# tungphambasement/DCNN

Measured on AMD Instinct MI355X. Metric: images/sec (whole node) ResNet-18 Tiny-ImageNet training at 1/2/4/8 MI355X, higher is better.
Workload: dtype bf16; 1 GPU; model=resnet18_tiny_imagenet, global_batch=256, per_gpu_batch=256, parallelism=dp1, optimizer=adam, hipgraph=True, engine=native (C++ host API)

## Files before the change

dcnn_amd/csrc/host/ops_gpu.hip:

```cpp
#include <hip/hip_runtime.h>

#include <algorithm>
#include <cmath>
#include <cstdio>
#include <cstdlib>
#include <cstring>
#include <map>
#include <mutex>
#include <stdexcept>
#include <string>
#include <unordered_map>
#include <vector>

#include "../kernels/api.h"
#include "dcnn/ops.hpp"
#include "dcnn/tensor.hpp"

#define HOST_HIP_CHECK(x)                                                                    \
  do {                                                                                       \
    hipError_t e_ = (x);                                                                     \
    if (e_ != hipSuccess) throw std::runtime_error(std::string(#x) + ": " + hipGetErrorString(e_)); \
  } while (0)

namespace dcnn {
// ... 739 lines not shown
  const GcArgs g = gc_args(s, groups);
  const int splits = dcnn::gconv_wgrad_splits(kBF16, g);
  wgrad_split(splits, (long)s.Co * s.KH * s.KW * (s.C / groups), s.Co, gw, gb,
              [&](float* slab, float* bslab) { dcnn::gconv_wgrad(kBF16, dy, x, slab, bslab, g, cur()); });
}

bool stem_ok(const ConvShape& s) {
  return s.KH == 3 && s.KW == 3 && s.SH == 1 && s.SW == 1 && s.PH == 1 && s.PW == 1 &&
         stem_supported(s.N, s.C, s.H, s.W, s.Co);
}

const float* stem_fwd(const float* x, const void* w, const float* bias, void* y, const ConvShape& s, int* stat_rows) {
  rec("stem_fwd", s, -1, {{"bias", bias != nullptr}, {"stats", stat_rows != nullptr}});
  StemArgs a{};
  a.x = x; a.w = w; a.w_bf16 = 1;
  a.ws[0] = 9l * s.C; a.ws[1] = 1; a.ws[2] = 3l * s.C; a.ws[3] = s.C;
  a.bias = bias; a.y = static_cast<bf16*>(y);
  a.N = s.N; a.Ci = s.C; a.H = s.H; a.W = s.W; a.Co = s.Co;
  if (stat_rows) {
    *stat_rows = stem_tiles_host(s.N, s.H, s.W);
    a.slab = static_cast<float*>(scratch(fwd_stats_slot(), (size_t)*stat_rows * 3 * s.Co * 4));
  }
  dcnn::stem_fwd(a, cur());
  return a.slab;
}

static void stem_wgrad_impl(const void* dy, const float* x, float* gw, float* gb, const ConvShape& s,
                            const StemBn* bn);

void stem_wgrad(const void* dy, const float* x, float* gw, float* gb, const ConvShape& s) {
  stem_wgrad_impl(dy, x, gw, gb, s, nullptr);
}

static std::pair<const float*, int> reduce_stats(int mode, const float* slab, int rows, int C);

void stem_wgrad_bn(const void* dy, const float* x, float* gw, float* gb, const ConvShape& s, const StemBn& bn) {
  stem_wgrad_impl(dy, x, gw, gb, s, &bn);
}

static void stem_wgrad_impl(const void* dy, const float* x, float* gw, float* gb, const ConvShape& s,
                            const StemBn* bn) {
  rec("stem_wgrad", s, -1, {{"bias", gb != nullptr}, {"deferred", g_defer}, {"bn", bn != nullptr}});
  std::pair<const float*, int> st{nullptr, 0};
  if (bn) st = reduce_stats(1, bn->slab, bn->rows, s.Co);
  const int blocks = bn ? stem_wgrad_blocks_bnt(s.N, s.H, s.W) : stem_wgrad_blocks(s.N, s.H, s.W);
  const long n = 9l * s.C * s.Co;
  wgrad_split(blocks, n, s.Co, gw, gb, [&](float* slab, float* bslab) {
    StemArgs a{};
    a.x = x; a.dy = static_cast<const bf16*>(dy); a.slab = slab; a.bias_slab = bslab;
    a.gs[0] = 9l * s.C; a.gs[1] = 1; a.gs[2] = 3l * s.C; a.gs[3] = s.C;
    a.n_slab = n;
    a.N = s.N; a.Ci = s.C; a.H = s.H; a.W = s.W; a.Co = s.Co;
    if (bn) {
      a.bn_x = static_cast<const bf16*>(bn->x); a.bn_mean = bn->mean; a.bn_istd = bn->istd; a.bn_gamma = bn->gamma;
      a.bn_sums = st.first; a.bn_parts = st.second; a.bn_count = (float)((long)s.N * s.H * s.W);
      a.bn_dgamma = bn->dgamma; a.bn_dbeta = bn->dbeta; a.bn_eval = bn->train ? 0 : 1;
    }
    dcnn::stem_wgrad(a, blocks, cur());
  });
}

void dense_fwd(const void* x, const void* w, const float* bias, void* y, int N, int In, int Out) {
  NtArgs a{static_cast<const bf16*>(x), static_cast<const bf16*>(w), y, N, Out, In, In, In, Out, kPlain, 0, 0, 0, 0,
           1, 1, 1, 1, 1, 1, 0, 0, bias, nullptr, nullptr, 0, 0};
  gemm_nt(a, cur());
}

void dense_dgrad(const void* dy, const void* w, void* dx, int N, int In, int Out) {
  bf16* wt = static_cast<bf16*>(scratch(W_T, (size_t)In * Out * 2));
  conv_weight_transpose(kBF16, w, wt, Out, 1, In, cur());
  NtArgs a{static_cast<const bf16*>(dy), wt, dx, N, In, Out, Out, Out, In, kPlain, 0, 0, 0, 0, 1, 1, 1, 1, 1, 1, 0, 0,
           nullptr, nullptr, nullptr, 0, 0};
  gemm_nt(a, cur());
}

void dense_wgrad(const void* dy, const void* x, float* gw, float* gb, int N, int In, int Out) {
  const int splits = gemm_tn_splits(Out, In, N);
  wgrad_split(splits, (long)Out * In, Out, gw, gb, [&](float* slab, float* bslab) {
    TnArgs a{static_cast<const bf16*>(dy), static_cast<const bf16*>(x), slab, bslab, Out, In, N, kPlain, 0, 0, 0, 0,
             1, 1, 1, 1, 1, 1, 0, 0, In, 0};
    gemm_tn(a, splits, cur());
  });
}

bool head_supported(const PoolShape& p, int Out) { return dcnn::head_supported(geom(p), Out); }

void head_fwd(const void* x, const void* w, const float* bias, void* pooled, void* y, const PoolShape& p, int Out) {
  dcnn::head_fwd(static_cast<const bf16*>(x), static_cast<const bf16*>(w), bias, static_cast<bf16*>(pooled),
                 static_cast<bf16*>(y), geom(p), Out, cur());
}

void head_bwd(const void* dy, const void* w, const void* pooled, void* dx, float* gw, float* gb, const PoolShape& p,
              int Out) {
  wgrad_split(head_bwd_splits(p.N, p.C, Out), (long)Out * p.C, Out, gw, gb, [&](float* slab, float* bslab) {
    dcnn::head_bwd(static_cast<const bf16*>(dy), static_cast<const bf16*>(w), static_cast<const bf16*>(pooled),
                   static_cast<bf16*>(dx), slab, bslab, geom(p), Out, cur());
  });
}

static std::pair<const float*, int> reduce_stats(int mode, const float* slab, int rows, int C) {
  const int parts = bn_stat_parts(rows);
  float* sums = static_cast<float*>(scratch(STAT_SUMS, (size_t)2 * C * 4));
  float* part = parts > 1 ? static_cast<float*>(scratch(STAT_PART, (size_t)parts * 3 * C * 4)) : nullptr;
  bn_stat_reduce(mode, slab, rows, C, sums, part, nullptr, cur());
  return {parts > 1 ? part : sums, parts};
}

void bn_fwd(const void* x, void* y, long R, int C, const float* g, const float* b, float eps, bool train,
            float* rmean, float* rvar, float momentum, float* smean, float* sistd, bool relu, const void* residual) {
  if (!train) {
    bn_apply(kBF16, x, y, R, C, nullptr, 1, (float)R, g, b, eps, residual, relu ? 1 : 0, smean, sistd, rmean, rvar,
             momentum, 1, cur());
    return;
  }
  const int rows = bn_partial_rows(R, C);
  float* slab = static_cast<float*>(scratch(STAT_SLAB, (size_t)rows * 3 * C * 4));
  bn_partial(kBF16, x, nullptr, nullptr, nullptr, nullptr, nullptr, R, C, slab, 0, nullptr, cur());
  const auto st = reduce_stats(0, slab, rows, C);
  bn_apply(kBF16, x, y, R, C, st.first, st.second, (float)R, g, b, eps, residual, relu ? 1 : 0, smean, sistd, rmean,
           rvar, momentum, 0, cur());
}

void bn_fwd_slab(const void* x, void* y, long R, int C, const float* slab, int rows, const float* g, const float* b,
                 float eps, float* rmean, float* rvar, float momentum, float* smean, float* sistd, bool relu,
                 const void* residual) {
  const auto st = reduce_stats(0, slab, rows, C);
  bn_apply(kBF16, x, y, R, C, st.first, st.second, (float)R, g, b, eps, residual, relu ? 1 : 0, smean, sistd, rmean,
           rvar, momentum, 0, cur());
}

void bn_bwd_slab(const void* dy, const void* x, void* dx, long R, int C, const float* mean, const float* istd,
                 const float* g, float* dg, float* db, bool train, const float* slab, int rows) {
  const auto st = reduce_stats(1, slab, rows, C);
  bn_bwd_apply(kBF16, dy, nullptr, x, dx, R, C, mean, istd, g, st.first, st.second, (float)R, dg, db, train ? 0 : 1, cur());
}

void bn_bwd(const void* dy, const void* x, void* dx, long R, int C, const float* mean, const float* istd,
            const float* g, float* dg, float* db, bool train, const void* yout, void* dy_out) {
  const int rows = bn_partial_rows(R, C);
  float* slab = static_cast<float*>(scratch(STAT_SLAB, (size_t)rows * 2 * C * 4));
  bn_partial(kBF16, x, dy, yout, dy_out, mean, istd, R, C, slab, 1, nullptr, cur());
  const auto st = reduce_stats(1, slab, rows, C);
  bn_bwd_apply(kBF16, dy, yout, x, dx, R, C, mean, istd, g, st.first, st.second, (float)R, dg, db, train ? 0 : 1, cur());
}

SecondaryStats::SecondaryStats() { t_secondary = true; }
SecondaryStats::~SecondaryStats() { t_secondary = false; }

BnRaw bn_stats_raw(const void* x, long R, int C, const float* slab, int rows) {
  if (slab != nullptr && rows > 0) return BnRaw{slab, rows};
  const int n = bn_partial_rows(R, C);
  float* s = static_cast<float*>(scratch(STAT_SLAB2, (size_t)n * 3 * C * 4));
  bn_partial(kBF16, x, nullptr, nullptr, nullptr, nullptr, nullptr, R, C, s, 0, nullptr, cur());
  return BnRaw{s, n};
}

bool bn_dual_ok(long R, int C) { return bn_apply_dual_supported(R, C); }

static void reduce_pair(int mode, const float* slab_a, int rows_a, const float* slab_b, int rows_b, int C,
                        std::pair<const float*, int>& a, std::pair<const float*, int>& b) {
  const int pa = bn_stat_parts(rows_a), pb = bn_stat_parts(rows_b);
  float* sa = static_cast<float*>(scratch(STAT_SUMS, (size_t)2 * C * 4));
  float* sb = static_cast<float*>(scratch(STAT_SUMS2, (size_t)2 * C * 4));
  float* qa = pa > 1 ? static_cast<float*>(scratch(STAT_PART, (size_t)pa * 3 * C * 4)) : nullptr;
  float* qb = pb > 1 ? static_cast<float*>(scratch(STAT_PART2, (size_t)pb * 3 * C * 4)) : nullptr;
  bn_stat_reduce2(mode, slab_a, rows_a, sa, qa, slab_b, rows_b, sb, qb, C, cur());
  a = {pa > 1 ? qa : sa, pa};
  b = {pb > 1 ? qb : sb, pb};
}

void bn_fwd_dual(const BnFwdSide& a, const BnFwdSide& b, void* y, long R, int C, bool relu, bool train) {
  std::pair<const float*, int> sa{nullptr, 1}, sb{nullptr, 1};
  if (train) reduce_pair(0, a.raw.slab, a.raw.rows, b.raw.slab, b.raw.rows, C, sa, sb);
  auto side = [&](const BnFwdSide& s, const std::pair<const float*, int>& st) {
    return BnSide{s.x,     st.first, st.second, (float)R, s.g,        s.b,    s.eps,
                  s.smean, s.sistd,  s.rmean,   s.rvar,   s.momentum, train ? 0 : 1};
  };
  if (!bn_apply_dual(side(a, sa), side(b, sb), y, R, C, relu ? 1 : 0, cur()))
    throw std::runtime_error("bn_fwd_dual: unsupported shape");
}

void bn_bwd_dual(const void* dy, const BnBwdSides& a, const float* slab_a, int rows_a, const BnBwdSides& b, long R,
                 int C) {
  const int rows_b = bn_partial_rows(R, C);
  float* slab_b = static_cast<float*>(scratch(STAT_SLAB, (size_t)rows_b * 2 * C * 4));
  bn_partial(kBF16, b.x, dy, nullptr, nullptr, b.mean, b.istd, R, C, slab_b, 1, nullptr, cur());
  std::pair<const float*, int> sa, sb;
  reduce_pair(1, slab_a, rows_a, slab_b, rows_b, C, sa, sb);
  auto side = [&](const BnBwdSides& s, const std::pair<const float*, int>& st) {
    return BnBwdSide{s.x, s.dx, s.mean, s.istd, s.g, st.first, st.second, (float)R, s.dg, s.db};
  };
  if (!bn_bwd_apply_dual(dy, side(a, sa), side(b, sb), R, C, cur()))
    throw std::runtime_error("bn_bwd_dual: unsupported shape");
}

bool bn_relu_maxpool_ok(const PoolShape& p) {
  const PoolGeom g = geom(p);
  return dcnn::bn_relu_maxpool_supported(g) && dcnn::maxpool_bwd_bnb_supported(g);
}

void bn_relu_maxpool(const void* x, void* y, uint8_t* idx, const PoolShape& p, const float* slab, int rows,
                     const float* g, const float* b, float eps, float* rmean, float* rvar, float momentum,
                     float* smean, float* sistd) {
  const long R = (long)p.N * p.H * p.W;
  if (slab == nullptr || rows <= 0) {
    rows = bn_partial_rows(R, p.C);
    float* s = static_cast<float*>(scratch(STAT_SLAB, (size_t)rows * 3 * p.C * 4));
    bn_partial(kBF16, x, nullptr, nullptr, nullptr, nullptr, nullptr, R, p.C, s, 0, nullptr, cur());
    slab = s;
  }
  const auto st = reduce_stats(0, slab, rows, p.C);
  dcnn::bn_relu_maxpool(static_cast<const bf16*>(x), static_cast<bf16*>(y), idx, geom(p), st.first, st.second,
                        (float)R, g, b, eps, smean, sistd, rmean, rvar, momentum, cur());
}

const float* maxpool_bwd_bnb(const void* dy, const uint8_t* idx, const void* ypool, const void* x, const float* mean,
                             const float* istd, void* dx, const PoolShape& p, int* rows) {
  const PoolGeom g = geom(p);
  *rows = maxpool_bwd_bnb_rows(g);
  float* slab = static_cast<float*>(scratch(BWD_STATS, (size_t)*rows * 2 * p.C * 4));
  dcnn::maxpool_bwd_bnb(static_cast<const bf16*>(dy), idx, static_cast<const bf16*>(ypool),
// ... 254 lines not shown
```

dcnn_amd/csrc/kernels/api.h:

```cpp
#pragma once
#include <hip/hip_runtime.h>
#include <stdint.h>

#include "fusion_plan.h"
#include "optim_segments.h"
typedef __bf16 bf16;

namespace dcnn {
struct BnbArgs {
  const bf16* y; const bf16* x; const float* mean; const float* istd;
  const float* gamma; const float* beta; int mask_x;
};
struct NtArgs {
  const bf16* A; const bf16* B; void* C;
  int M, N, K; int lda, ldb, ldc; int mode;
  int nb, sh, sw, cs, gh, gw; int kh, kw, strh, strw, padh, padw;
  const float* bias; const bf16* residual; float* stats; int out_f32; int relu;
};
struct TnArgs {
  const bf16* dY; const bf16* X; float* slab; float* bias_slab;
  int M, N, P; int mode; int nb, sh, sw, cs, gh, gw; int kh, kw, strh, strw, padh, padw; int ldx; int k_per_split;
};
struct G2Args {
  const bf16* A; const bf16* B; bf16* C;
// ... 117 lines not shown
void gemm_t2f(T2Args a, int splits, hipStream_t s);
int gemm_t2f_splits(int M, int N, int P);
void set_f32_mode(int mode);
int get_f32_mode();
void conv_weight_transpose_f32(const float* w, float* wt, int Co, int T_, int Ci, hipStream_t s);
void gemm_tn(TnArgs a, int splits, hipStream_t s);
int gemm_tn_splits(int M, int N, int P);
int gemm_tn_k_per_split(int P, int splits);
int gemm_tn_bias_rows(int M);
struct ConvRouteGeom {
  int N, C, H, W, Co, KH, KW, SH, SW, PH, PW, OH, OW, g1s_mode;
};
enum ConvRoute : int { ROUTE_GENERIC = 0, ROUTE_GEMM_G2 = 1, ROUTE_HALO = 2, ROUTE_G1S = 3, ROUTE_HALO_S2 = 4 };
int conv_fwd_route(ConvRouteGeom g);
int conv_dgrad_route(ConvRouteGeom g);
int conv_wgrad_route(ConvRouteGeom g);
void splitk_reduce(const float* slab, float* out, long n, int splits, int accumulate, hipStream_t s);
void splitk_reduce2(const float* slab, float* out, long n, const float* bslab, float* bout, long nb, int splits,
                    int accumulate, hipStream_t s);

constexpr int kMaxRed = 48;
struct RedEnt { const float* slab; float* out; long n; int splits, unit0, chunks, groups, vec, wpc; };
struct MultiRed { int count; RedEnt e[kMaxRed]; };
void multi_splitk_reduce(MultiRed t, hipStream_t s);

int bn_partial_rows(long R, int C);
void bn_partial(int dtype, const void* x, const void* dy, const void* yout, void* dy_out, const float* mean,
                const float* istd, long R, int C, float* slab, int mode, float* zero_sums, hipStream_t s);
int bn_stat_parts(int rows);
void bn_stat_reduce2(int mode, const float* slab, int rows, float* out, float* part, const float* slab2, int rows2,
                     float* out2, float* part2, int C, hipStream_t s);
void bn_stat_reduce(int mode, const float* slab, int rows, int C, float* out, float* part, unsigned* ticket,
                    hipStream_t s);
void bn_apply(int dtype, const void* x, void* y, long R, int C, const float* sums, int parts, float count, const float* gamma,
              const float* beta, float eps, const void* residual, int relu, float* save_mean, float* save_istd,
              float* run_mean, float* run_var, float momentum, int use_running, hipStream_t s);
struct BnSide {
  const void* x; const float* sums; int parts; float count; const float* gamma; const float* beta; float eps;
  float* save_mean; float* save_istd; float* run_mean; float* run_var; float momentum; int use_running;
};
bool bn_apply_dual(const BnSide& a, const BnSide& b, void* y, long R, int C, int relu, hipStream_t s);
bool bn_apply_dual_supported(long R, int C);
struct BnBwdSide {
  const void* x; void* dx; const float* mean; const float* istd; const float* gamma; const float* sums; int parts;
  float count; float* dgamma; float* dbeta;
};
bool bn_bwd_apply_dual(const void* dy, const BnBwdSide& a, const BnBwdSide& b, long R, int C, hipStream_t s);
void bn_bwd_apply(int dtype, const void* dy, const void* yout, const void* x, void* dx, long R, int C, const float* mean,
                  const float* istd, const float* gamma, const float* sums, int parts, float count, float* dgamma,
                  float* dbeta, int eval_mode, hipStream_t s);
bool bn_relu_maxpool_supported(PoolGeom g);
void bn_relu_maxpool(const bf16* x, bf16* y, uint8_t* idx, PoolGeom g, const float* sums, int parts, float count,
                     const float* gamma, const float* beta, float eps, float* save_mean, float* save_istd,
                     float* run_mean, float* run_var, float momentum, hipStream_t s);
void gn_fwd(int dtype, const void* x, void* y, int N, int HW, int C, int G, const float* gamma, const float* beta,
            float eps, float* save_mean, float* save_istd, hipStream_t s);
void gn_bwd(int dtype, const void* dy, const void* x, void* dx, int N, int HW, int C, int G, const float* gamma,
            const float* mean, const float* istd, float* dgamma, float* dbeta, float* aff, hipStream_t s);
bool ln_supported(int dt, long R, int C);
int ln_partial_rows(long R, int C);
long ln_workspace_bytes(long R, int C);
void ln_fwd(int dt, const void* x, void* y, long R, int C, const float* gamma, const float* beta, float eps,
            float* save_mean, float* save_rstd, hipStream_t s);
void ln_bwd(int dt, const void* dy, const void* x, void* dx, long R, int C, const float* gamma, const float* mean,
            const float* rstd, float* dgamma, float* dbeta, float* workspace, hipStream_t s);
void lscale_fwd(int dt, const void* x, const float* gamma, const void* residual, void* y, long R, int C,
// ... 130 lines not shown
```

dcnn_amd/csrc/kernels/bindings.cpp:

```cpp
#include <tuple>
#include <pybind11/pybind11.h>
#include <pybind11/stl.h>
#include <algorithm>
#include <array>
#include <vector>
#include <hip/hip_runtime.h>
#include <stdint.h>

namespace py = pybind11;
#include "api.h"


using namespace dcnn;
void bind_runtime(py::module_& m);
void bind_rccl(py::module_& m);
template <typename T>
static inline T P(uintptr_t x) { return reinterpret_cast<T>(x); }
static inline hipStream_t S(uintptr_t x) { return reinterpret_cast<hipStream_t>(x); }

using Ptr4 = std::array<uintptr_t, 4>;
static BnbArgs bnb_of(const Ptr4& b) {
  return BnbArgs{P<const bf16*>(b[0]), P<const bf16*>(b[1]), P<const float*>(b[2]), P<const float*>(b[3])};
}

// ... 242 lines not shown
                            unsigned b_bytes, int M, int N, int Pn, int splits, uintptr_t stream) {
    bind_gemm_t2(f32, dY, X, slab, bias_slab, a_bytes, b_bytes, M, N, Pn, M, N, 1, 1, 1, 1, 1, 1, {{0, 0}}, splits, stream);
  });
  m.def("gemm_t2_splits", &gemm_t2_splits);
  m.def("gemm_tn",
        [](uintptr_t dY, uintptr_t X, uintptr_t slab, uintptr_t bias_slab, int M, int N, int Pn, int mode, int nb,
           int sh, int sw, int cs, int gh, int gw, int kh, int kw, int strh, int strw, int padh, int padw, int ldx,
           int splits, uintptr_t stream) {
          TnArgs a{P<const bf16*>(dY), P<const bf16*>(X), P<float*>(slab), P<float*>(bias_slab), M, N, Pn, mode, nb, sh,
                   sw, cs, gh, gw, kh, kw, strh, strw, padh, padw, ldx, 0};
          gemm_tn(a, splits, S(stream));
        });
  m.def("gemm_tn_splits", &gemm_tn_splits);
  m.def("splitk_reduce", [](uintptr_t slab, uintptr_t out, long n, int splits, int acc, uintptr_t st) {
    splitk_reduce(P<const float*>(slab), P<float*>(out), n, splits, acc, S(st));
  });
  m.def("splitk_reduce2", [](uintptr_t slab, uintptr_t out, long n, uintptr_t bslab, uintptr_t bout, long nb,
                             int splits, int acc, uintptr_t st) {
    splitk_reduce2(P<const float*>(slab), P<float*>(out), n, P<const float*>(bslab), P<float*>(bout), nb, splits, acc,
                   S(st));
  });

  m.def("bn_partial_rows", &bn_partial_rows);
  m.def("bn_partial", [](int dt, uintptr_t x, uintptr_t dy, uintptr_t yout, uintptr_t dy_out, uintptr_t mean,
                         uintptr_t istd, long R, int C, uintptr_t slab, int mode, uintptr_t zero_sums, uintptr_t st) {
    bn_partial(dt, P<const void*>(x), P<const void*>(dy), P<const void*>(yout), P<void*>(dy_out),
               P<const float*>(mean), P<const float*>(istd), R, C, P<float*>(slab), mode, P<float*>(zero_sums), S(st));
  });
  m.def("bn_stat_parts", &bn_stat_parts);
  m.def("bn_stat_reduce", [](int mode, uintptr_t slab, int rows, int C, uintptr_t out, uintptr_t part, uintptr_t ticket,
                             uintptr_t st) {
    bn_stat_reduce(mode, P<const float*>(slab), rows, C, P<float*>(out), P<float*>(part), P<unsigned*>(ticket), S(st));
  });
  m.def("bn_apply", [](int dt, uintptr_t x, uintptr_t y, long R, int C, uintptr_t sums, int parts, float count,
                       uintptr_t gamma, uintptr_t beta, float eps, uintptr_t residual, int relu, uintptr_t save_mean,
                       uintptr_t save_istd, uintptr_t run_mean, uintptr_t run_var, float momentum, int use_running,
                       uintptr_t st) {
    bn_apply(dt, P<const void*>(x), P<void*>(y), R, C, P<const float*>(sums), parts, count, P<const float*>(gamma),
             P<const float*>(beta), eps, P<const void*>(residual), relu, P<float*>(save_mean), P<float*>(save_istd),
             P<float*>(run_mean), P<float*>(run_var), momentum, use_running, S(st));
  });
  using SideT = std::tuple<uintptr_t, uintptr_t, int, float, uintptr_t, uintptr_t, float, uintptr_t, uintptr_t, uintptr_t,
                           uintptr_t, float, int>;
  auto side = [](const SideT& t) {
    BnSide b{};
    b.x = P<const void*>(std::get<0>(t)); b.sums = P<const float*>(std::get<1>(t)); b.parts = std::get<2>(t);
    b.count = std::get<3>(t); b.gamma = P<const float*>(std::get<4>(t)); b.beta = P<const float*>(std::get<5>(t));
    b.eps = std::get<6>(t); b.save_mean = P<float*>(std::get<7>(t)); b.save_istd = P<float*>(std::get<8>(t));
    b.run_mean = P<float*>(std::get<9>(t)); b.run_var = P<float*>(std::get<10>(t)); b.momentum = std::get<11>(t);
    b.use_running = std::get<12>(t);
    return b;
  };
  m.def("bn_apply_dual", [side](SideT a, SideT b, uintptr_t y, long R, int C, int relu, uintptr_t st) {
    return bn_apply_dual(side(a), side(b), P<void*>(y), R, C, relu, S(st));
  });
  m.def("bn_apply_dual_supported", &bn_apply_dual_supported);
  using BSideT = std::tuple<uintptr_t, uintptr_t, uintptr_t, uintptr_t, uintptr_t, uintptr_t, int, float, uintptr_t,
                            uintptr_t>;
  auto bside = [](const BSideT& t) {
    BnBwdSide b{};
    b.x = P<const void*>(std::get<0>(t)); b.dx = P<void*>(std::get<1>(t)); b.mean = P<const float*>(std::get<2>(t));
    b.istd = P<const float*>(std::get<3>(t)); b.gamma = P<const float*>(std::get<4>(t));
    b.sums = P<const float*>(std::get<5>(t)); b.parts = std::get<6>(t); b.count = std::get<7>(t);
    b.dgamma = P<float*>(std::get<8>(t)); b.dbeta = P<float*>(std::get<9>(t));
    return b;
  };
// ... 415 lines not shown
```

dcnn_amd/csrc/kernels/norm.hip:

```cpp
#include <cstdlib>
#include <type_traits>

#include "common.h"
#include "api.h"

namespace dcnn {

template <typename T, int V>
struct VecIO;
template <>
struct VecIO<bf16, 8> {
  __device__ static __forceinline__ void load(const bf16* p, float* f) {
    unpack8(*reinterpret_cast<const uint4*>(p), f);
  }
  __device__ static __forceinline__ void store(bf16* p, const float* f) {
    *reinterpret_cast<uint4*>(p) = pack8(f);
  }
};
template <>
struct VecIO<float, 8> {
  __device__ static __forceinline__ void load(const float* p, float* f) {
    const float4 a = reinterpret_cast<const float4*>(p)[0], b = reinterpret_cast<const float4*>(p)[1];
    f[0] = a.x; f[1] = a.y; f[2] = a.z; f[3] = a.w; f[4] = b.x; f[5] = b.y; f[6] = b.z; f[7] = b.w;
  }
  __device__ static __forceinline__ void store(float* p, const float* f) {
    reinterpret_cast<float4*>(p)[0] = make_float4(f[0], f[1], f[2], f[3]);
    reinterpret_cast<float4*>(p)[1] = make_float4(f[4], f[5], f[6], f[7]);
  }
};
template <typename T>
struct VecIO1 {
  __device__ static __forceinline__ void load(const T* p, float* f) { f[0] = to_f(p[0]); }
  __device__ static __forceinline__ void store(T* p, const float* f) { p[0] = from_f<T>(f[0]); }
// ... 839 lines not shown
    o[0] = u.x; o[1] = u.y; o[2] = u.z; o[3] = u.w; o[4] = v.x; o[5] = v.y; o[6] = v.z; o[7] = v.w;
  };
  while (i < nv) {
    const unsigned inx = i + stride;
    uint4 nd{}, na{}, nb{};
    if (inx < nv) {
      nd = ldg16(dy + (size_t)inx * 8);
      na = ldg16(xa + (size_t)inx * 8);
      nb = ldg16(xb + (size_t)inx * 8);
    }
    const int c0 = (int)((cv & (cv - 1)) == 0 ? (i & (cv - 1)) : i % cv) * 8;
    float d[8];
    unpack8(vd, d);
#pragma unroll
    for (int side = 0; side < 2; ++side) {
      const float* ks = k + side * 4 * C;
      float A[8], B[8], M[8], D[8], xf[8], o[8];
      ld8(ks + c0, A);
      ld8(ks + C + c0, B);
      ld8(ks + 2 * C + c0, M);
      ld8(ks + 3 * C + c0, D);
      unpack8(side == 0 ? va : vb, xf);
#pragma unroll
      for (int v = 0; v < 8; ++v) o[v] = A[v] * d[v] + B[v] * (xf[v] - M[v]) + D[v];
      *reinterpret_cast<uint4*>((side == 0 ? da : db) + (size_t)i * 8) = pack8(o);
    }
    i = inx;
    vd = nd;
    va = na;
    vb = nb;
  }
}

bool bn_bwd_apply_dual(const void* dy, const BnBwdSide& a, const BnBwdSide& b, long R, int C, hipStream_t s) {
  if (!bn_apply_dual_supported(R, C)) return false;
  const unsigned nv = (unsigned)(R * C / 8);
  long g = (nv + 255) / 256;
  if (g > 1024) g = 1024;
  if (g < 1) g = 1;
  hipLaunchKernelGGL(bn_bwd_apply_dual_kernel, dim3((unsigned)g), dim3(256), 8 * C * sizeof(float), s,
                     static_cast<const bf16*>(dy), a, b, nv, C);
  DCNN_LAUNCH_CHECK();
  return true;
}



bool bn_apply_dual(const BnSide& a, const BnSide& b, void* y, long R, int C, int relu, hipStream_t s) {
  if (!bn_apply_dual_supported(R, C)) return false;
  const unsigned nv = (unsigned)(R * C / 8);
  long g = (nv + 255) / 256;
  if (g > 1024) g = 1024;
  if (g < 1) g = 1;
  hipLaunchKernelGGL(bn_apply_dual_kernel, dim3((unsigned)g), dim3(256), 4 * C * sizeof(float), s, a, b,
                     static_cast<bf16*>(y), nv, C, relu);
  DCNN_LAUNCH_CHECK();
  return true;
}

static void bn_v_launch_shape(long nv, int C, int* U, int* grid) {
  constexpr long g_cap = 1024;
  *U = 1;
  (void)C;
  const long cap = g_cap;
  long g = (nv + 256l * *U - 1) / (256l * *U);
  if (g > cap) g = cap;
  if (g < 1) g = 1;
  *grid = (int)g;
}

static bool g_bn_v = true;

void bn_set_vectorised(int on) { g_bn_v = on != 0; }

static bool bn_v_ok(long R, int C) { return g_bn_v && C % 8 == 0 && R * (long)C < (1l << 31); }

template <typename T>
__global__ void __launch_bounds__(256) gn_fwd_kernel(const T* __restrict__ x, T* __restrict__ y, int HW, int C,
                                                     int G, const float* __restrict__ gamma,
                                                     const float* __restrict__ beta, float eps,
                                                     float* __restrict__ save_mean, float* __restrict__ save_istd) {
  __shared__ float sh[16];
// ... 114 lines not shown
                       mode, zero_sums, s);
}

int bn_stat_parts(int rows) {
  const int per = g_stat_waves * kStatRW;
  return (rows + per - 1) / per;
}

void bn_stat_reduce2(int mode, const float* slab, int rows, float* out, float* part, const float* slab2, int rows2,
                     float* out2, float* part2, int C, hipStream_t s) {
  const int ny = bn_stat_parts(rows), ny2 = slab2 ? bn_stat_parts(rows2) : 0;
  if ((ny > 1 && !part) || (ny2 > 1 && !part2)) throw std::runtime_error("bn_stat_reduce: partials buffer required");
  const dim3 grid((unsigned)((C + 63) / 64), (unsigned)(ny > ny2 ? ny : ny2), slab2 ? 2u : 1u);
#define DCNN_SR(W)                                                                                           \
  if (g_stat_waves == W) {                                                                                   \
    if (mode == 0)                                                                                           \
      hipLaunchKernelGGL((bn_stat_reduce_kernel<0, W>), grid, dim3(64 * W), 0, s, slab, rows, C, part, nullptr, out, \
                         ny, slab2, rows2, part2, out2, ny2);                                                \
    else                                                                                                     \
      hipLaunchKernelGGL((bn_stat_reduce_kernel<1, W>), grid, dim3(64 * W), 0, s, slab, rows, C, part, nullptr, out, \
                         ny, slab2, rows2, part2, out2, ny2);                                                \
  }
  DCNN_SR(4) DCNN_SR(8) DCNN_SR(16)
#undef DCNN_SR
  DCNN_LAUNCH_CHECK();
}

void bn_stat_reduce(int mode, const float* slab, int rows, int C, float* out, float* part, unsigned* ticket,
                    hipStream_t s) {
  (void)ticket;
  bn_stat_reduce2(mode, slab, rows, out, part, nullptr, 0, nullptr, nullptr, C, s);
}

bool bn_relu_maxpool_supported(PoolGeom g) {
  return g.C % 8 == 0 && g.ph == g.sh && g.pw == g.sw && g.padh == 0 && g.padw == 0 && g.ph * g.pw <= 255 &&
         g.OH == g.H / g.ph && g.OW == g.W / g.pw;
}

void bn_relu_maxpool(const bf16* x, bf16* y, uint8_t* idx, PoolGeom g, const float* sums, int parts, float count,
                     const float* gamma, const float* beta, float eps, float* save_mean, float* save_istd,
                     float* run_mean, float* run_var, float momentum, hipStream_t s) {
  if (!bn_relu_maxpool_supported(g)) throw std::runtime_error("bn_relu_maxpool: unsupported geometry");
  const long total = (long)g.N * g.OH * g.OW * g.C / 8;
  auto k = (g.ph == 2 && g.pw == 2) ? bn_relu_maxpool_kernel<2> : bn_relu_maxpool_kernel<0>;
  hipLaunchKernelGGL(k, dim3(grid_for(total, 256, 2048)), dim3(256), 2 * g.C * sizeof(float), s,
                     x, y, idx, g, sums, parts, count, gamma, beta, eps, save_mean, save_istd, run_mean, run_var,
                     momentum);
  DCNN_LAUNCH_CHECK();
}

template <typename T>
static void bn_apply_t(const T* x, T* y, long R, int C, const float* sums, int parts, float count, const float* gamma,
                       const float* beta, float eps, const T* residual, int relu, float* save_mean,
                       float* save_istd, float* run_mean, float* run_var, float momentum, int use_running,
                       hipStream_t s) {
  const size_t shm = 2 * C * sizeof(float);
  if (bn_v_ok(R, C)) {
    int U, g;
    const unsigned nv = (unsigned)(R * C / 8);
    bn_v_launch_shape(nv, C, &U, &g);
#define DCNN_BNV(U_, RES_)                                                                                       \
  if (U == U_ && (residual != nullptr) == RES_)                                                                  \
    hipLaunchKernelGGL((bn_apply_v_kernel<T, U_, RES_>), dim3(g), dim3(256), shm, s, x, y, nv, C, sums, parts, count, \
                       gamma, beta, eps, residual, relu, save_mean, save_istd, run_mean, run_var, momentum, use_running);
    DCNN_BNV(1, false) DCNN_BNV(2, false) DCNN_BNV(4, false) DCNN_BNV(1, true) DCNN_BNV(2, true) DCNN_BNV(4, true)
#undef DCNN_BNV
    DCNN_LAUNCH_CHECK();
    return;
  }
  if (C % 8 == 0) {
    const int g = grid_for(R * C / 8, 256, 2048);
    hipLaunchKernelGGL((bn_apply_kernel<T, 8>), dim3(g), dim3(256), shm, s, x, y, R, C, sums, parts, count, gamma, beta,
                       eps, residual, relu, save_mean, save_istd, run_mean, run_var, momentum, use_running);
  } else {
    const int g = grid_for(R * C, 256, 2048);
    hipLaunchKernelGGL((bn_apply_kernel<T, 1>), dim3(g), dim3(256), shm, s, x, y, R, C, sums, parts, count, gamma, beta,
                       eps, residual, relu, save_mean, save_istd, run_mean, run_var, momentum, use_running);
  }
  DCNN_LAUNCH_CHECK();
}

void bn_apply(int dtype, const void* x, void* y, long R, int C, const float* sums, int parts, float count,
              const float* gamma, const float* beta, float eps, const void* residual, int relu, float* save_mean,
              float* save_istd, float* run_mean, float* run_var, float momentum, int use_running, hipStream_t s) {
  if (dtype == 0)
    bn_apply_t<float>((const float*)x, (float*)y, R, C, sums, parts, count, gamma, beta, eps, (const float*)residual,
                      relu, save_mean, save_istd, run_mean, run_var, momentum, use_running, s);
  else
    bn_apply_t<bf16>((const bf16*)x, (bf16*)y, R, C, sums, parts, count, gamma, beta, eps, (const bf16*)residual,
                     relu, save_mean, save_istd, run_mean, run_var, momentum, use_running, s);
}

template <typename T>
static void bn_bwd_apply_t(const T* dy, const T* yout, const T* x, T* dx, long R, int C, const float* mean,
                           const float* istd, const float* gamma, const float* sums, int parts, float count,
                           float* dgamma, float* dbeta, int eval_mode, hipStream_t s) {
  if (bn_v_ok(R, C)) {
    int U, g;
    const unsigned nv = (unsigned)(R * C / 8);
    bn_v_launch_shape(nv, C, &U, &g);
    const size_t shm4 = 4 * C * sizeof(float);
#define DCNN_BNBV(U_, MASK_)                                                                                      \
  if (U == U_ && (yout != nullptr) == MASK_)                                                                      \
    hipLaunchKernelGGL((bn_bwd_apply_v_kernel<T, U_, MASK_>), dim3(g), dim3(256), shm4, s, dy, yout, x, dx, nv, C, mean, \
                       istd, gamma, sums, parts, count, dgamma, dbeta, eval_mode);
    DCNN_BNBV(1, false) DCNN_BNBV(2, false) DCNN_BNBV(4, false) DCNN_BNBV(1, true) DCNN_BNBV(2, true) DCNN_BNBV(4, true)
#undef DCNN_BNBV
    DCNN_LAUNCH_CHECK();
    return;
  }
  const size_t shm = 5 * C * sizeof(float);
  if (C % 8 == 0) {
    const int g = grid_for(R * C / 8, 256, 2048);
    hipLaunchKernelGGL((bn_bwd_apply_kernel<T, 8>), dim3(g), dim3(256), shm, s, dy, yout, x, dx, R, C, mean, istd,
                       gamma, sums, parts, count, dgamma, dbeta, eval_mode);
  } else {
    const int g = grid_for(R * C, 256, 2048);
    hipLaunchKernelGGL((bn_bwd_apply_kernel<T, 1>), dim3(g), dim3(256), shm, s, dy, yout, x, dx, R, C, mean, istd,
                       gamma, sums, parts, count, dgamma, dbeta, eval_mode);
  }
  DCNN_LAUNCH_CHECK();
}

void bn_bwd_apply(int dtype, const void* dy, const void* yout, const void* x, void* dx, long R, int C,
                  const float* mean, const float* istd, const float* gamma, const float* sums, int parts, float count,
                  float* dgamma, float* dbeta, int eval_mode, hipStream_t s) {
  if (dtype == 0)
    bn_bwd_apply_t<float>((const float*)dy, (const float*)yout, (const float*)x, (float*)dx, R, C, mean, istd, gamma,
                          sums, parts, count, dgamma, dbeta, eval_mode, s);
// ... 33 lines not shown
```

Before: 91900 images/sec.

## Fold BN statistic reduction into apply kernels for small partial slabs

When the BatchNorm partial-statistics slab has few enough rows, the separate bn_stat_reduce launch is skipped. The raw slab is passed with a negative parts count, and new per-channel-slice apply kernels (forward, backward, single and dual) merge the slab rows in shared memory before applying. This removes one kernel launch and its global round trip per BN layer in forward and backward. In exchange, every block redundantly re-reduces the slab for its channel slice, and the apply grid is capped by channel slices times a workgroup limit, which may lower parallelism.

```diff
diff --git a/dcnn_amd/csrc/host/ops_gpu.hip b/dcnn_amd/csrc/host/ops_gpu.hip
--- a/dcnn_amd/csrc/host/ops_gpu.hip
+++ b/dcnn_amd/csrc/host/ops_gpu.hip
@@ -795,7 +795,7 @@
   stem_wgrad_impl(dy, x, gw, gb, s, nullptr);
 }
 
-static std::pair<const float*, int> reduce_stats(int mode, const float* slab, int rows, int C);
+static std::pair<const float*, int> reduce_stats(int mode, const float* slab, int rows, int C, long R = 0);
 
 void stem_wgrad_bn(const void* dy, const float* x, float* gw, float* gb, const ConvShape& s, const StemBn& bn) {
   stem_wgrad_impl(dy, x, gw, gb, s, &bn);
@@ -861,7 +861,8 @@
   });
 }
 
-static std::pair<const float*, int> reduce_stats(int mode, const float* slab, int rows, int C) {
+static std::pair<const float*, int> reduce_stats(int mode, const float* slab, int rows, int C, long R) {
+  if (R > 0 && bn_direct_ok(rows, R, C)) return {slab, -rows};
   const int parts = bn_stat_parts(rows);
   float* sums = static_cast<float*>(scratch(STAT_SUMS, (size_t)2 * C * 4));
   float* part = parts > 1 ? static_cast<float*>(scratch(STAT_PART, (size_t)parts * 3 * C * 4)) : nullptr;
@@ -879,7 +880,7 @@
   const int rows = bn_partial_rows(R, C);
   float* slab = static_cast<float*>(scratch(STAT_SLAB, (size_t)rows * 3 * C * 4));
   bn_partial(kBF16, x, nullptr, nullptr, nullptr, nullptr, nullptr, R, C, slab, 0, nullptr, cur());
-  const auto st = reduce_stats(0, slab, rows, C);
+  const auto st = reduce_stats(0, slab, rows, C, R);
   bn_apply(kBF16, x, y, R, C, st.first, st.second, (float)R, g, b, eps, residual, relu ? 1 : 0, smean, sistd, rmean,
            rvar, momentum, 0, cur());
 }
@@ -887,14 +888,14 @@
 void bn_fwd_slab(const void* x, void* y, long R, int C, const float* slab, int rows, const float* g, const float* b,
                  float eps, float* rmean, float* rvar, float momentum, float* smean, float* sistd, bool relu,
                  const void* residual) {
-  const auto st = reduce_stats(0, slab, rows, C);
+  const auto st = reduce_stats(0, slab, rows, C, R);
   bn_apply(kBF16, x, y, R, C, st.first, st.second, (float)R, g, b, eps, residual, relu ? 1 : 0, smean, sistd, rmean,
            rvar, momentum, 0, cur());
 }
 
 void bn_bwd_slab(const void* dy, const void* x, void* dx, long R, int C, const float* mean, const float* istd,
                  const float* g, float* dg, float* db, bool train, const float* slab, int rows) {
-  const auto st = reduce_stats(1, slab, rows, C);
+  const auto st = reduce_stats(1, slab, rows, C, R);
   bn_bwd_apply(kBF16, dy, nullptr, x, dx, R, C, mean, istd, g, st.first, st.second, (float)R, dg, db, train ? 0 : 1, cur());
 }
 
@@ -903,7 +904,7 @@
   const int rows = bn_partial_rows(R, C);
   float* slab = static_cast<float*>(scratch(STAT_SLAB, (size_t)rows * 2 * C * 4));
   bn_partial(kBF16, x, dy, yout, dy_out, mean, istd, R, C, slab, 1, nullptr, cur());
-  const auto st = reduce_stats(1, slab, rows, C);
+  const auto st = reduce_stats(1, slab, rows, C, R);
   bn_bwd_apply(kBF16, dy, yout, x, dx, R, C, mean, istd, g, st.first, st.second, (float)R, dg, db, train ? 0 : 1, cur());
 }
 
@@ -920,8 +921,13 @@
 
 bool bn_dual_ok(long R, int C) { return bn_apply_dual_supported(R, C); }
 
-static void reduce_pair(int mode, const float* slab_a, int rows_a, const float* slab_b, int rows_b, int C,
+static void reduce_pair(int mode, const float* slab_a, int rows_a, const float* slab_b, int rows_b, int C, long R,
                         std::pair<const float*, int>& a, std::pair<const float*, int>& b) {
+  if (bn_direct_pair_ok(mode, rows_a, rows_b, R, C)) {
+    a = {slab_a, -rows_a};
+    b = {slab_b, -rows_b};
+    return;
+  }
   const int pa = bn_stat_parts(rows_a), pb = bn_stat_parts(rows_b);
   float* sa = static_cast<float*>(scratch(STAT_SUMS, (size_t)2 * C * 4));
   float* sb = static_cast<float*>(scratch(STAT_SUMS2, (size_t)2 * C * 4));
@@ -934,7 +940,7 @@
 
 void bn_fwd_dual(const BnFwdSide& a, const BnFwdSide& b, void* y, long R, int C, bool relu, bool train) {
   std::pair<const float*, int> sa{nullptr, 1}, sb{nullptr, 1};
-  if (train) reduce_pair(0, a.raw.slab, a.raw.rows, b.raw.slab, b.raw.rows, C, sa, sb);
+  if (train) reduce_pair(0, a.raw.slab, a.raw.rows, b.raw.slab, b.raw.rows, C, R, sa, sb);
   auto side = [&](const BnFwdSide& s, const std::pair<const float*, int>& st) {
     return BnSide{s.x,     st.first, st.second, (float)R, s.g,        s.b,    s.eps,
                   s.smean, s.sistd,  s.rmean,   s.rvar,   s.momentum, train ? 0 : 1};
@@ -949,7 +955,7 @@
   float* slab_b = static_cast<float*>(scratch(STAT_SLAB, (size_t)rows_b * 2 * C * 4));
   bn_partial(kBF16, b.x, dy, nullptr, nullptr, b.mean, b.istd, R, C, slab_b, 1, nullptr, cur());
   std::pair<const float*, int> sa, sb;
-  reduce_pair(1, slab_a, rows_a, slab_b, rows_b, C, sa, sb);
+  reduce_pair(1, slab_a, rows_a, slab_b, rows_b, C, R, sa, sb);
   auto side = [&](const BnBwdSides& s, const std::pair<const float*, int>& st) {
     return BnBwdSide{s.x, s.dx, s.mean, s.istd, s.g, st.first, st.second, (float)R, s.dg, s.db};
   };
diff --git a/dcnn_amd/csrc/kernels/api.h b/dcnn_amd/csrc/kernels/api.h
--- a/dcnn_amd/csrc/kernels/api.h
+++ b/dcnn_amd/csrc/kernels/api.h
@@ -173,6 +173,10 @@
                      float* out2, float* part2, int C, hipStream_t s);
 void bn_stat_reduce(int mode, const float* slab, int rows, int C, float* out, float* part, unsigned* ticket,
                     hipStream_t s);
+int bn_direct_rows();
+bool bn_direct_ok(int rows, long R, int C);
+bool bn_direct_pair_ok(int mode, int rows_a, int rows_b, long R, int C);
+int bn_stat_route(int mode, const float* slab, int rows, long R, int C, float* out, float* part, hipStream_t s);
 void bn_apply(int dtype, const void* x, void* y, long R, int C, const float* sums, int parts, float count, const float* gamma,
               const float* beta, float eps, const void* residual, int relu, float* save_mean, float* save_istd,
               float* run_mean, float* run_var, float momentum, int use_running, hipStream_t s);
diff --git a/dcnn_amd/csrc/kernels/bindings.cpp b/dcnn_amd/csrc/kernels/bindings.cpp
--- a/dcnn_amd/csrc/kernels/bindings.cpp
+++ b/dcnn_amd/csrc/kernels/bindings.cpp
@@ -298,6 +298,13 @@
                              uintptr_t st) {
     bn_stat_reduce(mode, P<const float*>(slab), rows, C, P<float*>(out), P<float*>(part), P<unsigned*>(ticket), S(st));
   });
+  m.def("bn_direct_rows", &bn_direct_rows);
+  m.def("bn_direct_ok", &bn_direct_ok);
+  m.def("bn_direct_pair_ok", &bn_direct_pair_ok);
+  m.def("bn_stat_route", [](int mode, uintptr_t slab, int rows, long R, int C, uintptr_t out, uintptr_t part,
+                            uintptr_t st) {
+    return bn_stat_route(mode, P<const float*>(slab), rows, R, C, P<float*>(out), P<float*>(part), S(st));
+  });
   m.def("bn_apply", [](int dt, uintptr_t x, uintptr_t y, long R, int C, uintptr_t sums, int parts, float count,
                        uintptr_t gamma, uintptr_t beta, float eps, uintptr_t residual, int relu, uintptr_t save_mean,
                        uintptr_t save_istd, uintptr_t run_mean, uintptr_t run_var, float momentum, int use_running,
diff --git a/dcnn_amd/csrc/kernels/norm.hip b/dcnn_amd/csrc/kernels/norm.hip
--- a/dcnn_amd/csrc/kernels/norm.hip
+++ b/dcnn_amd/csrc/kernels/norm.hip
@@ -1,4 +1,6 @@
 #include <cstdlib>
+#include <stdexcept>
+#include <string>
 #include <type_traits>
 
 #include "common.h"
@@ -904,8 +906,292 @@
   }
 }
 
+constexpr int kDirectMaxRows = 8 * kStatRW;
+
+template <int MODE, int NS, int NW>
+__device__ __forceinline__ void direct_merge(const float* const* slab, const int* parts, int C, int c, bool cok,
+                                             StatAcc<MODE> (*red)[NW / NS][64]) {
+  constexpr int NV = MODE == 0 ? 3 : 2, WS = NW / NS;
+  static_assert(WS == 4 || WS == 8, "4 or 8 waves per slab");
+  const int lane = threadIdx.x & 63, w = threadIdx.x >> 6, sd = w / WS, wl = w % WS;
+  const float* __restrict__ src = slab[sd];
+  const int rows = -parts[sd];
+  StatAcc<MODE> t = StatAcc<MODE>::zero();
+  if (cok && rows > 0) {
+    t = stat_tree<MODE, kStatRW>(src, (long)NV * C, wl * kStatRW, min(rows, (wl + 1) * kStatRW), C, c);
+    if (WS == 4) {
+      StatAcc<MODE> u = StatAcc<MODE>::zero();
+      if (rows > 4 * kStatRW)
+        u = stat_tree<MODE, kStatRW>(src, (long)NV * C, (wl + 4) * kStatRW, min(rows, (wl + 5) * kStatRW), C, c);
+      t = t.merge(u);
+    }
+  } else if (WS == 4) {
+    t = t.merge(StatAcc<MODE>::zero());
+  }
+  red[sd][wl][lane] = t;
+#pragma unroll
+  for (int o = (WS == 4 ? 2 : 4); o > 0; o >>= 1) {
+    __syncthreads();
+    if (wl < o) red[sd][wl][lane] = red[sd][wl][lane].merge(red[sd][wl + o][lane]);
+  }
+  __syncthreads();
+}
+
+__device__ __forceinline__ void bn_slice_coeffs(const BnSide& b, int C, int c, bool first, float g, float be,
+                                                const StatAcc<0> (*red)[64], float* scale, float* shift) {
+  const int lane = threadIdx.x & 63;
+  float mean, var;
+  if (b.use_running) {
+    mean = b.run_mean[c];
+    var = b.run_var[c];
+  } else if (b.parts < 0) {
+    const StatAcc<0> t = red[0][lane];
+    mean = t.b;
+    var = t.a > 0.f ? t.c / t.a : 0.f;
+  } else {
+    read_stats<0>(b.sums, b.parts, C, c, mean, var);
+  }
+  const float istd = rsqrtf(var + b.eps);
+  if (!b.use_running && first) {
+    if (b.save_mean) { b.save_mean[c] = mean; b.save_istd[c] = istd; }
+    if (b.run_mean) {
+      const float unbiased = b.count > 1.f ? var * b.count / (b.count - 1.f) : var;
+      b.run_mean[c] = (1.f - b.momentum) * b.run_mean[c] + b.momentum * mean;
+      b.run_var[c] = (1.f - b.momentum) * b.run_var[c] + b.momentum * unbiased;
+    }
+  }
+  scale[lane] = g * istd;
+  shift[lane] = be - mean * g * istd;
+}
+
+template <typename T, int KIND, int NW>
+__global__ void __launch_bounds__(64 * NW) bn_apply_rows_kernel(BnSide a, BnSide b, const T* __restrict__ residual,
+                                                                T* __restrict__ y, unsigned npix, int C, int relu) {
+  constexpr int NS = KIND == 2 ? 2 : 1, WS = NW / NS;
+  __shared__ StatAcc<0> red[NS][WS][64];
+  __shared__ __attribute__((aligned(16))) float co[2 * NS][64];
+  using VT = Vec8<T>;
+  const T* __restrict__ xa = static_cast<const T*>(a.x);
+  const T* __restrict__ xr = KIND == 2 ? static_cast<const T*>(b.x) : residual;
+  const int v8 = (threadIdx.x & 7) * 8, cb = blockIdx.x * 64 + v8;
+  const bool vok = cb < C;
+  const unsigned pstride = gridDim.y * (8u * NW);
+  unsigned p = blockIdx.y * (8u * NW) + (threadIdx.x >> 3);
+  typename VT::type xv{}, rv{};
+  if (vok && p < npix) {
+    xv = VT::load(xa + (size_t)p * C + cb);
+    if (KIND != 0) rv = VT::load(xr + (size_t)p * C + cb);
+  }
+  const int c = blockIdx.x * 64 + (threadIdx.x & 63), sd = (threadIdx.x >> 6) / WS;
+  const BnSide& me = sd == 0 ? a : b;
+  const bool mine = (threadIdx.x >> 6) % WS == 0 && c < C;
+  float g = 1.f, be = 0.f;
+  if (mine) {
+    if (me.gamma) g = me.gamma[c];
+    if (me.beta) be = me.beta[c];
+  }
+  const float* const slabs[2] = {a.sums, b.sums};
+  const int parts[2] = {a.use_running ? 0 : a.parts, b.use_running ? 0 : b.parts};
+  direct_merge<0, NS, NW>(slabs, parts, C, c, c < C, red);
+  if (mine) bn_slice_coeffs(me, C, c, blockIdx.y == 0, g, be, red[sd], co[2 * sd], co[2 * sd + 1]);
+  __syncthreads();
+  if (!vok) return;
+  auto ld8 = [](const float* q, float* o) {
+    const float4 u = *reinterpret_cast<const float4*>(q), v = *reinterpret_cast<const float4*>(q + 4);
+    o[0] = u.x; o[1] = u.y; o[2] = u.z; o[3] = u.w; o[4] = v.x; o[5] = v.y; o[6] = v.z; o[7] = v.w;
+  };
+  float sc[8], sf[8], sb[8], hb[8];
+  ld8(co[0] + v8, sc);
+  ld8(co[1] + v8, sf);
+  if (KIND == 2) {
+    ld8(co[2 * (NS - 1)] + v8, sb);
+    ld8(co[2 * (NS - 1) + 1] + v8, hb);
+  }
+  while (p < npix) {
+    const unsigned pn = p + pstride;
+    typename VT::type xn{}, rn{};
+    if (pn < npix) {
+      xn = VT::load(xa + (size_t)pn * C + cb);
+      if (KIND != 0) rn = VT::load(xr + (size_t)pn * C + cb);
+    }
+    float f[8], r[8];
+    VT::unpack(xv, f);
+    if (KIND != 0) VT::unpack(rv, r);
+#pragma unroll
+    for (int v = 0; v < 8; ++v) {
+      float t = f[v] * sc[v] + sf[v];
+      if (KIND == 1) t += r[v];
+      if (KIND == 2) t += (float)(T)(r[v] * sb[v] + hb[v]);
+      if (relu) t = fmaxf(t, 0.f);
+      f[v] = t;
+    }
+    VT::store(y + (size_t)p * C + cb, f);
+    p = pn;
+    xv = xn;
+    if (KIND != 0) rv = rn;
+  }
+}
+
+__device__ __forceinline__ void bn_bwd_slice_coeffs(const BnBwdSide& b, int eval_mode, int C, int c, bool first,
+                                                    float g, float is, float m, const StatAcc<1> (*red)[64],
+                                                    float* ca, float* cbm, float* cm, float* cd) {
+  const int lane = threadIdx.x & 63;
+  float sdy = 0.f, sdyx = 0.f;
+  if (b.sums) {
+    if (b.parts < 0) {
+      sdy = red[0][lane].a;
+      sdyx = red[0][lane].b;
+    } else {
+      read_stats<1>(b.sums, b.parts, C, c, sdy, sdyx);
+    }
+  }
+  const float a = g * is;
+  ca[lane] = a;
+  cbm[lane] = eval_mode ? 0.f : -a * is * (sdyx / b.count);
+  cm[lane] = m;
+  cd[lane] = eval_mode ? 0.f : -a * (sdy / b.count);
+  if (first && b.sums) {
+    if (b.dgamma) b.dgamma[c] += sdyx;
+    if (b.dbeta) b.dbeta[c] += sdy;
+  }
+}
+
+template <typename T, int KIND, int NW>
+__global__ void __launch_bounds__(64 * NW) bn_bwd_apply_rows_kernel(const T* __restrict__ dy,
+                                                                    const T* __restrict__ yout, BnBwdSide a,
+                                                                    BnBwdSide b, unsigned npix, int C, int eval_mode) {
+  constexpr int NS = KIND == 2 ? 2 : 1, WS = NW / NS;
+  __shared__ StatAcc<1> red[NS][WS][64];
+  __shared__ __attribute__((aligned(16))) float co[4 * NS][64];
+  using VT = Vec8<T>;
+  const T* __restrict__ xa = static_cast<const T*>(a.x);
+  const T* __restrict__ x2 = KIND == 2 ? static_cast<const T*>(b.x) : yout;
+  T* __restrict__ da = static_cast<T*>(a.dx);
+  T* __restrict__ db = static_cast<T*>(b.dx);
+  const int v8 = (threadIdx.x & 7) * 8, cb = blockIdx.x * 64 + v8;
+  const bool vok = cb < C;
+  const unsigned pstride = gridDim.y * (8u * NW);
+  unsigned p = blockIdx.y * (8u * NW) + (threadIdx.x >> 3);
+  typename VT::type dv{}, xv{}, tv{};
+  if (vok && p < npix) {
+    dv = VT::load(dy + (size_t)p * C + cb);
+    xv = VT::load(xa + (size_t)p * C + cb);
+    if (KIND != 0) tv = VT::load(x2 + (size_t)p * C + cb);
+  }
+  const int c = blockIdx.x * 64 + (threadIdx.x & 63), sd = (threadIdx.x >> 6) / WS;
+  const BnBwdSide& me = sd == 0 ? a : b;
+  const bool mine = (threadIdx.x >> 6) % WS == 0 && c < C;
+  float g = 1.f, is = 0.f, m = 0.f;
+  if (mine) {
+    if (me.gamma) g = me.gamma[c];
+    is = me.istd[c];
+    m = me.mean[c];
+  }
+  const float* const slabs[2] = {a.sums, b.sums};
+  const int parts[2] = {a.sums ? a.parts : 0, b.sums ? b.parts : 0};
+  direct_merge<1, NS, NW>(slabs, parts, C, c, c < C, red);
+  if (mine)
+    bn_bwd_slice_coeffs(me, eval_mode, C, c, blockIdx.y == 0, g, is, m, red[sd], co[4 * sd], co[4 * sd + 1],
+                        co[4 * sd + 2], co[4 * sd + 3]);
+  __syncthreads();
+  if (!vok) return;
+  auto ld8 = [](const float* q, float* o) {
+    const float4 u = *reinterpret_cast<const float4*>(q), v = *reinterpret_cast<const float4*>(q + 4);
+    o[0] = u.x; o[1] = u.y; o[2] = u.z; o[3] = u.w; o[4] = v.x; o[5] = v.y; o[6] = v.z; o[7] = v.w;
+  };
+  float A[NS][8], B[NS][8], M[NS][8], D[NS][8];
+#pragma unroll
+  for (int s = 0; s < NS; ++s) {
+    ld8(co[4 * s + 0] + v8, A[s]);
+    ld8(co[4 * s + 1] + v8, B[s]);
+    ld8(co[4 * s + 2] + v8, M[s]);
+    ld8(co[4 * s + 3] + v8, D[s]);
+  }
+  while (p < npix) {
+    const unsigned pn = p + pstride;
+    typename VT::type dn{}, xn{}, tn{};
+    if (pn < npix) {
+      dn = VT::load(dy + (size_t)pn * C + cb);
+      xn = VT::load(xa + (size_t)pn * C + cb);
+      if (KIND != 0) tn = VT::load(x2 + (size_t)pn * C + cb);
+    }
+    float d[8], t[8];
+    VT::unpack(dv, d);
+    if (KIND != 0) VT::unpack(tv, t);
+    if (KIND == 1) {
+#pragma unroll
+      for (int v = 0; v < 8; ++v) d[v] = t[v] > 0.f ? d[v] : 0.f;
+    }
+#pragma unroll
+    for (int s = 0; s < NS; ++s) {
+      float xf[8], o[8];
+      if (s == 0) {
+        VT::unpack(xv, xf);
+      } else {
+#pragma unroll
+        for (int v = 0; v < 8; ++v) xf[v] = t[v];
+      }
+#pragma unroll
+      for (int v = 0; v < 8; ++v) o[v] = A[s][v] * d[v] + B[s][v] * (xf[v] - M[s][v]) + D[s][v];
+      VT::store((s == 0 ? da : db) + (size_t)p * C + cb, o);
+    }
+    p = pn;
+    dv = dn;
+    xv = xn;
+    if (KIND != 0) tv = tn;
+  }
+}
+
+static bool bn_v_ok(long R, int C);
+
+static const int g_direct_rows = [] {
+  const char* e = std::getenv("DCNN_BN_DIRECT_ROWS");
+  const int v = e && *e ? std::atoi(e) : kDirectMaxRows;
+  return g_stat_waves != 8 || v < 0 ? 0 : (v > kDirectMaxRows ? kDirectMaxRows : v);
+}();
+static const int g_direct_wgs = [] {
+  const char* e = std::getenv("DCNN_BN_DIRECT_WGS");
+  const int v = e && *e ? std::atoi(e) : 512;
+  return v < 1 ? 1 : v;
+}();
+
+int bn_direct_rows() { return g_direct_rows; }
+
+bool bn_direct_ok(int rows, long R, int C) { return rows >= 1 && rows <= g_direct_rows && bn_v_ok(R, C); }
+
+bool bn_direct_pair_ok(int mode, int rows_a, int rows_b, long R, int C) {
+  const int lim = mode == 0 ? 4 * kStatRW : kDirectMaxRows;
+  return rows_a <= lim && rows_b <= lim && bn_direct_ok(rows_a, R, C) && bn_direct_ok(rows_b, R, C) &&
+         bn_apply_dual_supported(R, C);
+}
+
+static void bn_rows_check(const char* what, int parts, long R, int C) {
+  if (parts >= 0) return;
+  if (-parts > kDirectMaxRows || g_stat_waves != 8 || !bn_v_ok(R, C))
+    throw std::invalid_argument(std::string(what) + ": a raw statistics slab (parts < 0) needs at most " +
+                                std::to_string(kDirectMaxRows) + " rows, the 8-wave reduce order and the "
+                                "vectorised kernels (C % 8 == 0, fewer than 2^31 elements)");
+}
+
+static dim3 bn_rows_grid(long R, int C, int nw) {
+  const int slices = (C + 63) / 64;
+  long p = (R + 8 * nw - 1) / (8 * nw), cap = (long)g_direct_wgs * 4 / nw / slices;
+  if (cap < 1) cap = 1;
+  if (p > cap) p = cap;
+  if (p < 1) p = 1;
+  return dim3((unsigned)slices, (unsigned)p);
+}
+
 bool bn_bwd_apply_dual(const void* dy, const BnBwdSide& a, const BnBwdSide& b, long R, int C, hipStream_t s) {
   if (!bn_apply_dual_supported(R, C)) return false;
+  if (a.parts < 0 || b.parts < 0) {
+    bn_rows_check("bn_bwd_apply_dual", a.parts, R, C);
+    bn_rows_check("bn_bwd_apply_dual", b.parts, R, C);
+    hipLaunchKernelGGL((bn_bwd_apply_rows_kernel<bf16, 2, 8>), bn_rows_grid(R, C, 8), dim3(512), 0, s,
+                       static_cast<const bf16*>(dy), static_cast<const bf16*>(nullptr), a, b, (unsigned)R, C, 0);
+    DCNN_LAUNCH_CHECK();
+    return true;
+  }
   const unsigned nv = (unsigned)(R * C / 8);
   long g = (nv + 255) / 256;
   if (g > 1024) g = 1024;
@@ -920,6 +1206,14 @@
 
 bool bn_apply_dual(const BnSide& a, const BnSide& b, void* y, long R, int C, int relu, hipStream_t s) {
   if (!bn_apply_dual_supported(R, C)) return false;
+  if (a.parts < 0 || b.parts < 0) {
+    bn_rows_check("bn_apply_dual", a.parts, R, C);
+    bn_rows_check("bn_apply_dual", b.parts, R, C);
+    hipLaunchKernelGGL((bn_apply_rows_kernel<bf16, 2, 8>), bn_rows_grid(R, C, 8), dim3(512), 0, s, a, b,
+                       static_cast<const bf16*>(nullptr), static_cast<bf16*>(y), (unsigned)R, C, relu);
+    DCNN_LAUNCH_CHECK();
+    return true;
+  }
   const unsigned nv = (unsigned)(R * C / 8);
   long g = (nv + 255) / 256;
   if (g > 1024) g = 1024;
@@ -1100,6 +1394,12 @@
   bn_stat_reduce2(mode, slab, rows, out, part, nullptr, 0, nullptr, nullptr, C, s);
 }
 
+int bn_stat_route(int mode, const float* slab, int rows, long R, int C, float* out, float* part, hipStream_t s) {
+  if (bn_direct_ok(rows, R, C)) return -rows;
+  bn_stat_reduce2(mode, slab, rows, out, part, nullptr, 0, nullptr, nullptr, C, s);
+  return bn_stat_parts(rows);
+}
+
 bool bn_relu_maxpool_supported(PoolGeom g) {
   return g.C % 8 == 0 && g.ph == g.sh && g.pw == g.sw && g.padh == 0 && g.padw == 0 && g.ph * g.pw <= 255 &&
          g.OH == g.H / g.ph && g.OW == g.W / g.pw;
@@ -1123,6 +1423,18 @@
                        float* save_istd, float* run_mean, float* run_var, float momentum, int use_running,
                        hipStream_t s) {
   const size_t shm = 2 * C * sizeof(float);
+  if (parts < 0 && !use_running) {
+    bn_rows_check("bn_apply", parts, R, C);
+    const BnSide a{x, sums, parts, count, gamma, beta, eps, save_mean, save_istd, run_mean, run_var, momentum, 0};
+#define DCNN_BNR(KIND_, NW_)                                                                                  \
+  if ((residual ? 1 : 0) == KIND_ && (-parts > 4 * kStatRW ? 8 : 4) == NW_)                                   \
+    hipLaunchKernelGGL((bn_apply_rows_kernel<T, KIND_, NW_>), bn_rows_grid(R, C, NW_), dim3(64 * NW_), 0, s, a, \
+                       BnSide{}, residual, y, (unsigned)R, C, relu);
+    DCNN_BNR(0, 4) DCNN_BNR(0, 8) DCNN_BNR(1, 4) DCNN_BNR(1, 8)
+#undef DCNN_BNR
+    DCNN_LAUNCH_CHECK();
+    return;
+  }
   if (bn_v_ok(R, C)) {
     int U, g;
     const unsigned nv = (unsigned)(R * C / 8);
@@ -1163,6 +1475,18 @@
 static void bn_bwd_apply_t(const T* dy, const T* yout, const T* x, T* dx, long R, int C, const float* mean,
                            const float* istd, const float* gamma, const float* sums, int parts, float count,
                            float* dgamma, float* dbeta, int eval_mode, hipStream_t s) {
+  if (parts < 0 && sums) {
+    bn_rows_check("bn_bwd_apply", parts, R, C);
+    const BnBwdSide a{x, dx, mean, istd, gamma, sums, parts, count, dgamma, dbeta};
+#define DCNN_BNBR(KIND_, NW_)                                                                                   \
+  if ((yout ? 1 : 0) == KIND_ && (-parts > 4 * kStatRW ? 8 : 4) == NW_)                                          \
+    hipLaunchKernelGGL((bn_bwd_apply_rows_kernel<T, KIND_, NW_>), bn_rows_grid(R, C, NW_), dim3(64 * NW_), 0, s, dy, \
+                       yout, a, BnBwdSide{}, (unsigned)R, C, eval_mode);
+    DCNN_BNBR(0, 4) DCNN_BNBR(0, 8) DCNN_BNBR(1, 4) DCNN_BNBR(1, 8)
+#undef DCNN_BNBR
+    DCNN_LAUNCH_CHECK();
+    return;
+  }
   if (bn_v_ok(R, C)) {
     int U, g;
     const unsigned nv = (unsigned)(R * C / 8);
```

Result: no change. 92670 images/sec, median of 6 (+0.8%).
